# HarmoniaLeo/FRLW-EvD

Hardware: AMD Instinct MI355X
Metric: TAF encode throughput (Mevents/s) (higher is better)
Workload: dtype f32

## Files before the change

### frlw-evd_amd/csrc/taf_column.h

```cpp
#pragma once
#include "frlw_common.h"
#include "taf_plan.h"

namespace {
using namespace frlw;
#define LDS_FENCE() asm volatile("" ::: "memory")
#define LDS_BARRIER() asm volatile("s_waitcnt lgkmcnt(0)\n\ts_barrier" ::: "memory")


struct CmP {
    const uint32_t *dir;
    int n_chunks;
    const uint32_t *rec;
    int TB;
    int chunk_ev;
    uint32_t *hot_start;
    uint32_t *hot_seg0;
    uint32_t *segdesc;
    int max_segs;
};

template <int NT>
__device__ __forceinline__ uint32_t col_load(const CmP &m, const SeqTab &S, int s, int b, uint32_t *L, uint32_t *D, uint32_t *wsum)
{
    constexpr int NWV = NT / kWave;
    const int tid = threadIdx.x, lane = tid & 63, wv = tid >> 6;
    const int c0 = S.chunk0[s], C = S.chunk0[s + 1] - c0;
    const uint32_t out0 = (uint32_t)(S.ev0[s] - S.ev0[0]);
    uint32_t carry = 0;
    for (int cb = 0; cb < C; cb += NT) {
        const int c = cb + tid;
        const uint32_t v = m.dir[(long long)b * m.n_chunks + (c0 + (c < C ? c : C - 1))];
        const uint32_t e = c < C ? v : 0u, cnt = e >> 16;
        const uint32_t inc = wave_incl_scan(cnt);
        if (lane == kWave - 1) wsum[wv] = inc;
        __syncthreads();
        uint32_t run = carry + inc - cnt, total = 0;
#pragma unroll
        for (int k = 0; k < NWV; ++k) { if (k < wv) run += wsum[k]; total += wsum[k]; }
        if (c < C) {
            L[c] = run;
            D[c] = out0 + (uint32_t)c * (uint32_t)m.chunk_ev + (e & 0xffffu) - run;
        }
        carry += total;
        __syncthreads();
    }
    if (tid == 0) L[C] = carry;
    __syncthreads();
    return (uint32_t)__builtin_amdgcn_readfirstlane((int)carry);
}

__device__ __forceinline__ uint32_t col_load_wave(const CmP &m, const SeqTab &S, int s, int b, uint32_t *L, uint32_t *D)
{
    const int lane = threadIdx.x & 63;
    const int c0 = S.chunk0[s], C = S.chunk0[s + 1] - c0;
    const uint32_t out0 = (uint32_t)(S.ev0[s] - S.ev0[0]);
    uint32_t n = 0;
    for (int cb = 0; cb < C; cb += kWave) {
        const int c = cb + lane;
        const uint32_t v = m.dir[(long long)b * m.n_chunks + (c0 + (c < C ? c : C - 1))];
        const uint32_t e = c < C ? v : 0u, cnt = e >> 16;
        const uint32_t inc = wave_incl_scan(cnt), run = n + inc - cnt;
        if (c < C) { L[c] = run; D[c] = out0 + (uint32_t)c * (uint32_t)m.chunk_ev + (e & 0xffffu) - run; }
        n += (uint32_t)__builtin_amdgcn_readlane((int)inc, kWave - 1);
    }
    if (lane == 0) L[C] = n;
    return n;
}

template <int NG, int RU, class Sink>
__device__ __forceinline__ void col_gather(const uint32_t *L, const uint32_t *D, int C, int g16, int l16, const uint32_t *rec, Sink sink)
{
    for (int cc0 = g16; cc0 < C; cc0 += NG * RU) {
        uint32_t v[RU], at[RU], cnt[RU];
#pragma unroll
        for (int u = 0; u < RU; ++u) {
            const int c = cc0 + NG * u, cc = c < C ? c : C - 1;
            const uint32_t lo = L[cc];
            cnt[u] = c < C ? L[cc + 1] - lo : 0u;
            at[u] = lo;
            v[u] = rec[D[cc] + lo + ((uint32_t)l16 < cnt[u] ? (uint32_t)l16 : 0u)];
        }
#pragma unroll
        for (int u = 0; u < RU; ++u) {
            if ((uint32_t)l16 < cnt[u]) sink(at[u] + l16, v[u]);
            if (cnt[u] > 16u) {
                const int c = cc0 + NG * u;
                const uint32_t d = D[c], lo = L[c];
                for (uint32_t j = 16u + l16; j < cnt[u]; j += 16u) sink(lo + j, rec[d + lo + j]);
            }
        }
    }
}

template <int NT>
__device__ __forceinline__ void col_index(const uint32_t *L, int C, uint32_t lo, uint32_t hi, uint16_t *idx)
{
    for (int c = threadIdx.x; c < C; c += NT) {
        const uint32_t a = L[c] > lo ? L[c] : lo, z = L[c + 1] < hi ? L[c + 1] : hi;
        for (uint32_t i = (a + 15u) & ~15u; i < z; i += 16u) idx[(i - lo) >> 4] = (uint16_t)c;
    }
}

__device__ __forceinline__ uint32_t col_addr(const uint32_t *L, const uint32_t *D, uint32_t c, uint32_t i);

__device__ __forceinline__ uint32_t col_addr_wave(const uint32_t *L, const uint32_t *D, const uint16_t *idx, uint32_t lo, uint32_t r0,
                                                  uint32_t ric, uint32_t nr)
{
    if (r0 >= nr) return D[0] + L[0];
    const uint32_t i0 = lo + r0, last = lo + (r0 + 63u < nr ? r0 + 63u : nr - 1u);
    uint32_t cs = (uint32_t)__builtin_amdgcn_readfirstlane((int)idx[r0 >> 4]);
    uint32_t lnext = (uint32_t)__builtin_amdgcn_readfirstlane((int)L[cs + 1]);
    while (lnext <= i0) { ++cs; lnext = (uint32_t)__builtin_amdgcn_readfirstlane((int)L[cs + 1]); }
    if (lnext > last) return (uint32_t)__builtin_amdgcn_readfirstlane((int)D[cs]) + lo + ric;
    return col_addr(L, D, idx[ric >> 4], lo + ric);
}

__device__ __forceinline__ uint32_t col_addr(const uint32_t *L, const uint32_t *D, uint32_t c, uint32_t i)
{
    c += L[c + 1] <= i ? 1u : 0u;
    c += L[c + 1] <= i ? 1u : 0u;
    if (__builtin_expect(__ballot(L[c + 1] <= i) != 0ull, 0))
        while (L[c + 1] <= i) ++c;
    return D[c] + i;
}
}
```

### frlw-evd_amd/csrc/taf_partition.h

```cpp
#pragma once
#include "taf_decode.h"
#include <stddef.h>

namespace {
__host__ __device__ inline uint32_t whole_max_of(int pairs) { return pairs < kFewPairs ? (uint32_t)kSplitSeg : (uint32_t)kSplitWhole; }
__host__ __device__ inline uint32_t split_segments(uint32_t n, uint32_t whole_max) { return n > whole_max ? (n + kSplitSeg - 1) / kSplitSeg : 0u; }

struct HistSpan {
    long long first;
    long long begin, end;
    long long t0;
};

__device__ __forceinline__ HistSpan hist_span(const FastGeom &G, const SeqTab &S, int chunk, int n_chunks)
{
    HistSpan L;
    L.begin = L.end = L.first = 0;
    L.t0 = 0;
    if (chunk >= n_chunks) return L;
    const int s = seq_of_chunk(S, chunk);
    L.t0 = S.t0[s];
    L.begin = S.ev0[s] + (long long)(chunk - S.chunk0[s]) * G.chunk_ev;
    L.end = L.begin + G.chunk_ev < S.ev0[s + 1] ? L.begin + G.chunk_ev : S.ev0[s + 1];
    if (L.end < L.begin) L.end = L.begin;
    L.first = L.begin - (long long)((reinterpret_cast<uintptr_t>(G.data + L.begin) >> 3) & 1u);
    if (L.first < 0) L.first = L.begin;
    return L;
}

__device__ __forceinline__ uint32_t hist_pairs(const HistSpan &L)
{
    long long cover = L.end - L.first;
    if (cover > 2ll * (kMaxBpw / 2) * kFT) cover = 2ll * (kMaxBpw / 2) * kFT;
    return (uint32_t)(cover >> 1);
}

__device__ __forceinline__ void hist_issue(const FastGeom &G, const HistSpan &L, uint4 (&v)[kMaxBpw / 2])
{
    const uint32_t pairs = hist_pairs(L);
    if (pairs > 0) {
        const uint4 *src = (const uint4 *)(G.data + L.first);
#pragma unroll
        for (int j = 0; j < kMaxBpw / 2; ++j) {
            const uint32_t pj = (uint32_t)(j * kFT) + threadIdx.x;
            v[j] = src[pj < pairs ? pj : pairs - 1u];
        }
    }
}

template <bool HAS_MAP, bool EV = false, bool SIMPLE = false>
__global__ __launch_bounds__(kFT) __attribute__((amdgpu_waves_per_eu(8, 8))) void kf_hist(FastGeom G, SeqTab S, uint32_t *counts,
                                                                                         int32_t *errs, float *tlut_w, int n_chunks)
{
    extern __shared__ uint32_t lds[];
    uint32_t *hist = lds;
    __shared__ int serr;
    const int tid = threadIdx.x;
    for (int b = tid; b < G.T; b += kFT) hist[b] = 0;
    if (tid == 0) serr = 0;
    int mul_err = 0;
    if (EV) {
        const double den = (double)G.win, rcp = G.rcp;
        for (long long r = (long long)blockIdx.x * kFT + tid; r <= (long long)G.win; r += (long long)gridDim.x * kFT) {
            const float exact = (float)((double)r / den);
            if ((float)((double)r * rcp) != exact) mul_err = ST_MULBAD;
            tlut_w[r] = exact;
        }
    } else if (tlut_w) {
        const double den = (double)G.win + 1e-8, rcp = G.rcp;
        for (long long r = (long long)blockIdx.x * kFT + tid; r <= (long long)G.win; r += (long long)gridDim.x * kFT) {
            const float exact = (float)((double)r / den);
            if ((float)((double)r * rcp) != exact) mul_err = ST_MULBAD;
            tlut_w[r] = exact - 1.0f;
        }
    }
    uint4 cur[kMaxBpw / 2], nxt[kMaxBpw / 2];
    HistSpan Lc, Ln = hist_span(G, S, (int)blockIdx.x, n_chunks);
    hist_issue(G, Ln, nxt);
    if (mul_err) atomicOr(&serr, mul_err);
    __syncthreads();
    for (int chunk = (int)blockIdx.x; chunk < n_chunks; chunk += (int)gridDim.x) {
        Lc = Ln;
#pragma unroll
        for (int j = 0; j < kMaxBpw / 2; ++j) cur[j] = nxt[j];
        Ln = hist_span(G, S, chunk + (int)gridDim.x, n_chunks);
        hist_issue(G, Ln, nxt);
        int err = 0;
        const uint32_t pairs = hist_pairs(Lc);
        const bool skip_first = Lc.first != Lc.begin;
#pragma unroll
        for (int j = 0; j < kMaxBpw / 2; ++j) {
            const uint32_t pj = (uint32_t)(j * kFT + tid);
            if (pj < pairs && !(skip_first && pj == 0u)) {
                const FastEv o = fast_decode<HAS_MAP, EV, SIMPLE>(G, make_uint2(cur[j].x, cur[j].y), Lc.t0);
                err |= o.err;
                if (o.tile >= 0) atomicAdd(&hist[o.tile], 1u);
            }
            if (pj < pairs) {
                const FastEv o = fast_decode<HAS_MAP, EV, SIMPLE>(G, make_uint2(cur[j].z, cur[j].w), Lc.t0);
                err |= o.err;
                if (o.tile >= 0) atomicAdd(&hist[o.tile], 1u);
            }
        }
        if (tid == 0 && Lc.end > Lc.begin && Lc.first + 2ll * pairs < Lc.end) {
            const FastEv o = fast_decode<HAS_MAP, EV, SIMPLE>(G, G.data[Lc.end - 1], Lc.t0);
            err |= o.err;
            if (o.tile >= 0) atomicAdd(&hist[o.tile], 1u);
        }
        if (err) atomicOr(&serr, err);
        __syncthreads();
        uint32_t *row = counts + (long long)chunk * G.T;
        for (int b = tid; b < G.T; b += kFT) { row[b] = hist[b]; hist[b] = 0u; }
        if (tid == 0) { errs[chunk] = serr; serr = 0; }
        __syncthreads();
    }
}

__device__ __forceinline__ void slabscan_one(const SeqTab &S, uint32_t *counts, int T, uint32_t *slabtot, int slab, int b)
{
    const int s = seq_of(S.slab0, S.n_seq, slab);
    const int c0 = S.chunk0[s] + (slab - S.slab0[s]) * kFastSlab, cend = S.chunk0[s + 1];
    uint32_t v[kFastSlab];
#pragma unroll
    for (int k = 0; k < kFastSlab; ++k) v[k] = (c0 + k < cend) ? counts[(long long)(c0 + k) * T + b] : 0u;
    uint32_t run = 0;
#pragma unroll
    for (int k = 0; k < kFastSlab; ++k) {
        const uint32_t t = v[k];
        v[k] = run;
        run += t;
    }
#pragma unroll
    for (int k = 0; k < kFastSlab; ++k)
        if (c0 + k < cend) counts[(long long)(c0 + k) * T + b] = v[k];
    slabtot[(long long)slab * T + b] = run;
}
__global__ __launch_bounds__(kWave) void kf_slabscan(SeqTab S, uint32_t *counts, int T, uint32_t *slabtot)
{
    const int b = blockIdx.x * kWave + threadIdx.x;
    if (b < T) slabscan_one(S, counts, T, slabtot, blockIdx.y, b);
}

constexpr int kInlineSlabScan = 8192;
__global__ __launch_bounds__(kFT) void kf_tilescan(SeqTab S, uint32_t *slabtot, int T, uint32_t *base, uint32_t *seg0,
                                                   FastHeader *hdr, const int32_t *errs, int chunks, uint32_t *counts_inline,
                                                   int slabs_inline, int no_segments)
{
    if (counts_inline) {
        for (int i = threadIdx.x; i < slabs_inline * T; i += kFT) slabscan_one(S, counts_inline, T, slabtot, i / T, i % T);
        __syncthreads();
    }
    __shared__ uint32_t tot[kMaxPairs];
    __shared__ uint32_t wsum[kFW], wsum2[kFW];
    const int tid = threadIdx.x, lane = tid & 63, wv = tid >> 6;
    const int pairs = S.n_seq * T;
    if (tid == 0) { hdr->status = 0; hdr->filtered_tiles = 0u; hdr->mul_bad = 0u; }
    if (tid < kMaxSeq) hdr->wmask[tid] = 0ull;
    __syncthreads();
    {
        int e = 0;
        for (int c = tid; c < chunks; c += kFT) e |= errs[c];
        if (e & ~ST_MULBAD) atomicOr(&hdr->status, e & ~ST_MULBAD);
        if (e & ST_MULBAD) hdr->mul_bad = 1u;
    }
    const uint32_t whole_max = no_segments ? 0xffffffffu : whole_max_of(pairs);
    uint32_t carry = 0, scarry = 0;
    for (int p0 = 0; p0 < pairs; p0 += kMaxPairs) {
        const int np = pairs - p0 < kMaxPairs ? pairs - p0 : kMaxPairs;
        for (int idx = tid; idx < np; idx += kFT) {
            const int gi = p0 + idx, s = gi / T, b = gi - s * T;
            uint32_t run = 0;
            const int sl1 = S.slab0[s + 1];
            for (int sl = S.slab0[s]; sl < sl1; sl += 8) {
                uint32_t v[8];
#pragma unroll
                for (int k = 0; k < 8; ++k) v[k] = sl + k < sl1 ? slabtot[(long long)(sl + k) * T + b] : 0u;
#pragma unroll
                for (int k = 0; k < 8; ++k) {
                    if (sl + k < sl1) slabtot[(long long)(sl + k) * T + b] = run;
                    run += v[k];
                }
            }
            tot[idx] = run;
        }
        __syncthreads();
        const int per = (np + kFT - 1) / kFT;
        const int b0 = tid * per;
        int b1 = b0 + per;
        if (b1 > np) b1 = np;
        uint32_t sum = 0, ssum = 0;
        for (int b = b0; b < b1; ++b) { sum += tot[b]; ssum += split_segments(tot[b], whole_max); }
        uint32_t inc = sum, sinc = ssum;
#pragma unroll
        for (int off = 1; off < kWave; off <<= 1) {
            const uint32_t v = __shfl_up(inc, off), v2 = __shfl_up(sinc, off);
            if (lane >= off) { inc += v; sinc += v2; }
        }
        if (lane == kWave - 1) { wsum[wv] = inc; wsum2[wv] = sinc; }
        __syncthreads();
        uint32_t pre = 0, spre = 0, all = 0, sall = 0;
        for (int k = 0; k < kFW; ++k) {
            if (k < wv) { pre += wsum[k]; spre += wsum2[k]; }
            all += wsum[k]; sall += wsum2[k];
        }
        uint32_t run = carry + pre + inc - sum, srun = scarry + spre + sinc - ssum;
        for (int b = b0; b < b1; ++b) {
            base[p0 + b] = run;
            seg0[p0 + b] = srun;
            run += tot[b];
            srun += split_segments(tot[b], whole_max);
        }
        carry += all;
        scarry += sall;
        __syncthreads();
    }
    if (tid == 0) { base[pairs] = carry; seg0[pairs] = scarry; }
    if (tid == 0) fold_sticky_status(hdr, hdr->status);
}

template <bool HAS_MAP, bool EV = false, bool SIMPLE = false>
__global__ __launch_bounds__(kFT) void kf_scatter(FastGeom G, SeqTab S, const uint32_t *counts, const uint32_t *slabtot,
                                                  const uint32_t *base, uint32_t *records, FastHeader *hdr)
{
    extern __shared__ uint32_t lds[];
    const int T = G.T;
    uint32_t *wcnt_all = lds;
    uint32_t *loff = wcnt_all + (size_t)kFW * T;
    uint32_t *stage = loff + ((T + 2) & ~1);
    uint16_t *stile = (uint16_t *)(stage + G.chunk_ev);
    __shared__ uint32_t wtot[kFW];
    __shared__ unsigned long long wg_seen;
    const int tid = threadIdx.x, lane = tid & 63, wv = tid >> 6;
    const int chunk = (int)chunk_of_block(blockIdx.x, gridDim.x);
    const int s = seq_of_chunk(S, chunk);
    uint32_t *wcnt = wcnt_all + (size_t)wv * T;
    for (int b = tid; b < kFW * T; b += kFT) wcnt_all[b] = 0;
    if (tid == 0) wg_seen = 0ull;
    __syncthreads();

    const long long chunk_begin = S.ev0[s] + (long long)(chunk - S.chunk0[s]) * G.chunk_ev;
    const long long wave_begin = chunk_begin + (long long)wv * G.run;
    const long long left = S.ev0[s + 1] - wave_begin;
    const uint32_t nloc = left < (long long)G.run ? (uint32_t)(left < 0 ? 0 : left) : (uint32_t)G.run;
    const long long t0 = S.t0[s];
    uint2 q[kMaxBpw];
    if (nloc > 0) {
        const uint2 *src = G.data + wave_begin;
#pragma unroll
        for (int j = 0; j < kMaxBpw; ++j) {
            const uint32_t i = (uint32_t)(j * kWave + lane);
            q[j] = src[i < nloc ? i : nloc - 1u];
        }
    }
    const int slab = S.slab0[s] + (chunk - S.chunk0[s]) / kFastSlab;
    const int tcl = tid < T ? tid : 0;
    const uint32_t gs_a = base[s * T + tcl], gs_b = slabtot[(long long)slab * T + tcl], gs_c = counts[(long long)chunk * T + tcl];
    uint32_t where[kMaxBpw], word[kMaxBpw];
    unsigned long long wseen = 0ull;
#pragma unroll
    for (int j = 0; j < kMaxBpw; ++j) {
        where[j] = 0xffffffffu;
        word[j] = 0u;
        if (j < G.bpw) {
            const uint32_t i = (uint32_t)(j * kWave + lane);
            if (i < nloc) {
                const FastEv o = fast_decode<HAS_MAP, EV, SIMPLE>(G, q[j], t0);
                if (o.tile >= 0) {
                    const uint32_t r = atomicAdd(&wcnt[o.tile], 1u);
                    where[j] = ((uint32_t)o.tile << 16) | r;
                    word[j] = o.word;
                    wseen |= 1ull << o.window;
                }
            }
        }
    }
    __syncthreads();
    uint32_t mine = 0;
    for (int b = tid; b < T; b += kFT) {
        uint32_t run = 0;
#pragma unroll
        for (int w = 0; w < kFW; ++w) {
            const uint32_t v = wcnt_all[(size_t)w * T + b];
            wcnt_all[(size_t)w * T + b] = run;
            run += v;
        }
        mine = run;
    }
    const uint32_t inc = wave_incl_scan(mine);
    if (lane == kWave - 1) wtot[wv] = inc;
    __syncthreads();
    uint32_t pre = 0, total = 0;
#pragma unroll
    for (int k = 0; k < kFW; ++k) { if (k < wv) pre += wtot[k]; total += wtot[k]; }
    if (tid < T) loff[tid] = pre + inc - mine;
    __syncthreads();
#pragma unroll
    for (int j = 0; j < kMaxBpw; ++j) {
        if (j < G.bpw && where[j] != 0xffffffffu) {
            const uint32_t b = where[j] >> 16;
            const uint32_t slot = loff[b] + wcnt[b] + (where[j] & 0xffffu);
            stage[slot] = word[j];
            stile[slot] = (uint16_t)b;
        }
    }
#pragma unroll
    for (int off = 32; off >= 1; off >>= 1) {
        const unsigned lo = __shfl_xor((unsigned)wseen, off), hi = __shfl_xor((unsigned)(wseen >> 32), off);
        wseen |= ((unsigned long long)hi << 32) | lo;
    }
    if (lane == 0 && wseen) atomicOr(&wg_seen, wseen);
    __syncthreads();
    if (tid < T) loff[tid] = (gs_a + gs_b + gs_c) - loff[tid];
    __syncthreads();
    for (uint32_t qi = tid; qi < total; qi += kFT) records[loff[stile[qi]] + qi] = stage[qi];
    if (tid == 0) {
        const unsigned long long m = wg_seen;
        const unsigned long long have = __hip_atomic_load(&hdr->wmask[s], __ATOMIC_RELAXED, __HIP_MEMORY_SCOPE_AGENT);
        if (m & ~have) atomicOr(&hdr->wmask[s], m);
    }
}


#ifndef FRLW_SCATTER_AHEAD
#define FRLW_SCATTER_AHEAD 4
#endif
#if defined(FRLW_WALK_PROF) || defined(FRLW_SCAT_PROF)
constexpr int kProfWgs = 131072;
__device__ unsigned long long g_walk_prof[kProfWgs * 9];
#define XPROF(i) do { const unsigned long long t_ = __builtin_amdgcn_s_memtime(); pd_[i] += t_ - tp_; tp_ = t_; } while (0)
#define XPROF_INIT() unsigned long long tp_ = __builtin_amdgcn_s_memtime(), pd_[9] = {0, 0, 0, 0, 0, 0, 0, 0, 0}
#define XPROF_END() do { if (threadIdx.x == 0 && blockIdx.x < kProfWgs) for (int i_ = 0; i_ < 9; ++i_) g_walk_prof[blockIdx.x * 9 + i_] += pd_[i_]; } while (0)
#endif
#ifdef FRLW_WALK_PROF
#define WPROF(i) XPROF(i)
#define WPROF_INIT() XPROF_INIT()
#define WPROF_END() XPROF_END()
#else
#define WPROF(i) do { } while (0)
#define WPROF_INIT() do { } while (0)
#define WPROF_END() do { } while (0)
#endif
#ifdef FRLW_SCAT_PROF
#define SPROF(i) XPROF(i)
#define SPROF_INIT() XPROF_INIT()
#define SPROF_END() XPROF_END()
#define SPROF_DRAIN() asm volatile("s_waitcnt vmcnt(0)" ::: "memory")
#else
#define SPROF(i) do { } while (0)
#define SPROF_INIT() do { } while (0)
#define SPROF_END() do { } while (0)
#define SPROF_DRAIN() do { } while (0)
#endif
template <bool HAS_MAP, bool EV = false, bool SIMPLE = false, int MAXB = kMaxBpw, int SAE = 0>
__global__ __launch_bounds__(kFT) __attribute__((amdgpu_waves_per_eu(MAXB > kMaxBpw ? 4 : 8, MAXB > kMaxBpw ? 4 : 8))) void kf_scatter_cm(FastGeom G, SeqTab S, uint32_t *dir, uint32_t *records, FastHeader *hdr, float *tlut_w,
                                                     uint32_t epoch)
{
    extern __shared__ uint32_t lds[];
    const int T = G.T;
    uint32_t *wcnt_all = lds;
    uint32_t *loff = wcnt_all + (size_t)kFW * T;
    uint32_t *stage = loff + ((T + 2) & ~1);
    __shared__ uint32_t wtot[kFW];
    __shared__ unsigned long long wg_seen;
    __shared__ int serr;
    constexpr bool LEAN = SIMPLE && !EV && !HAS_MAP && SAE == 0;
    const int tid = threadIdx.x, lane = tid & 63, wv = LEAN ? __builtin_amdgcn_readfirstlane(tid >> 6) : tid >> 6;
    SPROF_INIT();
    const int chunk = (int)chunk_of_block(blockIdx.x, gridDim.x);
    const int s = seq_of_chunk(S, chunk);
    uint32_t *wcnt = wcnt_all + (size_t)wv * T;
    for (int b = tid; b < kFW * T; b += kFT) wcnt_all[b] = 0;
    if (tid == 0) { wg_seen = 0ull; serr = 0; }
    if (blockIdx.x == 0 && epoch != 0u) {
        uint32_t *h32 = (uint32_t *)hdr;
        for (int i = tid; i < (int)(offsetof(FastHeader, epoch) / 4); i += kFT) h32[i] = 0u;
        if (tid == 0) {
            uint32_t *sw = (uint32_t *)((char *)hdr + kStallOffset);
            const uint32_t was = __hip_atomic_load(sw, __ATOMIC_RELAXED, __HIP_MEMORY_SCOPE_AGENT);
            if (was != 0u && was != epoch) atomicCAS(sw, was, 0u);
        }
        __threadfence();
        __syncthreads();
        if (tid == 0) __hip_atomic_store(&hdr->epoch, epoch, __ATOMIC_RELEASE, __HIP_MEMORY_SCOPE_AGENT);
    }

    const long long chunk_begin = S.ev0[s] + (long long)(chunk - S.chunk0[s]) * G.chunk_ev;
    const long long wave_begin = chunk_begin + (long long)wv * G.run;
    const long long left = S.ev0[s + 1] - wave_begin;
    const uint32_t nloc = left < (long long)G.run ? (uint32_t)(left < 0 ? 0 : left) : (uint32_t)G.run;
    const long long t0 = S.t0[s];
    constexpr int kAhead = MAXB > FRLW_SCATTER_AHEAD ? FRLW_SCATTER_AHEAD : MAXB;
    uint2 q[MAXB];
    const uint2 *src = G.data + wave_begin;
    const uint32_t last = nloc - 1u;
    if (nloc > 0) {
#pragma unroll
        for (int j = 0; j < kAhead; ++j) q[j] = src[min((uint32_t)(j * kWave + lane), last)];
    }
    int pre_err = 0;
    if (tlut_w) {
        const double den = EV ? (double)G.win : (double)G.win + 1e-8, rcp = G.rcp;
        bool bad = false;
        for (long long r = (long long)blockIdx.x * kFT + tid; r <= (long long)G.win; r += (long long)gridDim.x * kFT) {
            const float exact = (float)((double)r / den);
            bad |= (float)((double)r * rcp) != exact;
            tlut_w[r] = EV ? exact : exact - 1.0f;
        }
        if (bad) pre_err = ST_MULBAD;
    }
    asm volatile("s_waitcnt lgkmcnt(0)\n\ts_barrier" ::: "memory");
    SPROF(0);
    SPROF(1);
    constexpr bool FASTBLK = LEAN && MAXB > kMaxBpw;
    uint32_t where[MAXB], word[MAXB];
    unsigned long long wseen = 0ull;
    uint32_t wseen32 = 0u;
    int err = pre_err;
    const uint32_t t0lo = (uint32_t)t0;
    const uint32_t nfast = FASTBLK && G.m24 && G.n_windows <= 32 && t0lo <= ~G.span ? nloc >> 6 : 0u;
#pragma unroll
    for (int j = 0; j < MAXB; ++j) {
        where[j] = 0xffffffffu;
        word[j] = 0u;
        if (j + kAhead < MAXB) {
            if (nloc > 0 && j + kAhead < G.bpw)
                q[j + kAhead] = src[min((uint32_t)((j + kAhead) * kWave + lane), last)];
            asm volatile("" ::: "memory");
        }
        bool fast = false;
        uint32_t fx = 0u, fy = 0u, frel = 0u;
        if (FASTBLK && (uint32_t)j < nfast) {
            fx = q[j].y & 16383u; fy = (q[j].y >> 14) & 16383u; frel = q[j].x - t0lo;
            fast = (__builtin_amdgcn_ballot_w64(fx >= (uint32_t)G.W) | __builtin_amdgcn_ballot_w64(fy >= (uint32_t)G.H_full) |
                    __builtin_amdgcn_ballot_w64(frel >= G.span)) == 0ull;
        }
        if (fast) {
            uint32_t tile, w, z;
            simple_taf_fields_valid(G, fx, fy, (q[j].y >> 28) & 1u, frel, tile, w, z);
            const uint32_t r = atomicAdd(&wcnt[tile], 1u);
            wseen32 |= 1u << z;
            word[j] = w;
            where[j] = (tile << 16) | r;
        } else if (j < G.bpw) {
            const uint32_t i = (uint32_t)(j * kWave + lane);
            if (LEAN) {
                if (nloc > 0) {
                    int x = (int)(q[j].y & 16383u), y = (int)((q[j].y >> 14) & 16383u);
                    const uint32_t p = (q[j].y >> 28) & 1u;
                    const bool ib = !fast_alias(G, x, y);
                    uint32_t tile, w, z;
                    const bool sb = !simple_taf_fields<!FASTBLK>(G, x, y, p, q[j].x, t0lo, tile, w, z);
                    const bool live = i < nloc, ok = live && !ib && !sb;
                    if (live && !ok) err |= ib ? ST_INDEX : ST_SPAN;
                    uint32_t r = 0u;
                    if (ok) {
                        r = atomicAdd(&wcnt[tile], 1u);
                        wseen |= 1ull << z;
                    }
                    where[j] = ok ? (tile << 16) | r : 0xffffffffu;
                    word[j] = w;
                }
            } else if (i < nloc) {
                const FastEv o = fast_decode<HAS_MAP, EV, SIMPLE, SAE>(G, q[j], t0);
                err |= o.err;
                if (o.tile >= 0) {
                    const uint32_t r = atomicAdd(&wcnt[o.tile], 1u);
                    where[j] = ((uint32_t)o.tile << 16) | r;
                    word[j] = SAE ? ((uint32_t)(wave_begin - S.ev0[s] + (long long)i + 1) << kCellBits) | (o.word & (uint32_t)(kCells - 1)) : o.word;
                    wseen |= 1ull << o.window;
                }
            }
        }
    }
    wseen |= wseen32;
    if (err) atomicOr(&serr, err);
    SPROF(2);
    __syncthreads();
    SPROF(3);
    uint32_t mine = 0;
    uint32_t pv[kFW];
    {
        const int b = tid < T ? tid : 0;
#pragma unroll
        for (int w = 0; w < kFW; ++w) {
            pv[w] = mine;
            mine += wcnt_all[(size_t)w * T + b];
        }
        if (tid >= T) mine = 0u;
    }
    const uint32_t inc = wave_incl_scan(mine);
    if (lane == kWave - 1) wtot[wv] = inc;
    __syncthreads();
    uint32_t pre = 0, total = 0;
#pragma unroll
    for (int k = 0; k < kFW; ++k) { if (k < wv) pre += wtot[k]; total += wtot[k]; }
    const uint32_t my_off = pre + inc - mine;
    if (tid < T) {
#pragma unroll
        for (int w = 0; w < kFW; ++w) wcnt_all[(size_t)w * T + tid] = pv[w] + my_off;
        dir[(long long)tid * (long long)gridDim.x + chunk] = (mine << 16) | my_off;
    }
    __syncthreads();
    SPROF(4);
#pragma unroll
    for (int j = 0; j < MAXB; ++j) {
        if (j < G.bpw && where[j] != 0xffffffffu) {
            const uint32_t b = where[j] >> 16;
            stage[wcnt[b] + (where[j] & 0xffffu)] = word[j];
        }
    }
#pragma unroll
    for (int off = 32; off >= 1; off >>= 1) {
        const unsigned lo = __shfl_xor((unsigned)wseen, off), hi = __shfl_xor((unsigned)(wseen >> 32), off);
        wseen |= ((unsigned long long)hi << 32) | lo;
    }
    if (lane == 0 && wseen) atomicOr(&wg_seen, wseen);
    __syncthreads();
    SPROF(5);
    uint32_t *dst = records + (chunk_begin - S.ev0[0]);
    uint32_t q4 = 0u;
    if (((reinterpret_cast<uintptr_t>(dst) | reinterpret_cast<uintptr_t>(stage)) & 15u) == 0u) {
        q4 = total & ~3u;
        for (uint32_t qi = 4u * tid; qi < q4; qi += 4u * kFT) *reinterpret_cast<uint4 *>(dst + qi) = *reinterpret_cast<const uint4 *>(stage + qi);
    }
    for (uint32_t qi = q4 + tid; qi < total; qi += kFT) dst[qi] = stage[qi];
    SPROF(6);
    SPROF_DRAIN();
    SPROF(7);
    SPROF_END();
    if (tid == 0) {
        if (epoch != 0u) {
            uint32_t polls = 0u;
            while (__hip_atomic_load(&hdr->epoch, __ATOMIC_ACQUIRE, __HIP_MEMORY_SCOPE_AGENT) != epoch) {
                if (++polls > (1u << 22)) break;
                __builtin_amdgcn_s_sleep(2);
            }
            if (polls > (1u << 22)) {
                atomicExch((uint32_t *)((char *)hdr + kStallOffset), epoch);
                fold_sticky_status(hdr, ST_STALL);
                return;
            }
        }
        const unsigned long long m = wg_seen;
        const unsigned long long have = __hip_atomic_load(&hdr->wmask[s], __ATOMIC_RELAXED, __HIP_MEMORY_SCOPE_AGENT);
        if (m & ~have) atomicOr(&hdr->wmask[s], m);
        const int e = serr;
        if (e & ~ST_MULBAD) { atomicOr(&hdr->status, e & ~ST_MULBAD); fold_sticky_status(hdr, e & ~ST_MULBAD); }
        if (e & ST_MULBAD) hdr->mul_bad = 1u;
    }
}
}
```

### frlw-evd_amd/csrc/taf_split.h

```cpp
#pragma once
#include "taf_blocktab.h"
#include "taf_column.h"
#include "taf_partition.h"
#include <type_traits>

namespace {
struct TileP {
    int H, W, twl, thl, tiles_x, T, K, n_windows, wb, flip;
    uint32_t win;
    const uint32_t *rec;
    uint32_t *rec2;
    const uint32_t *base;
    uint32_t *sub;
    uint32_t *sub_end;
    const uint32_t *seg0;
    uint32_t *segcnt;
    int pairs;
    int direct;
    int seg_grid;
    uint32_t tile_max;
    const float *tlut;
    const uint32_t *leaky_thr;
    FastHeader *hdr;
    double rcp;
    float *state;
    float *view_f32;
    uint8_t *out_u8;
    uint32_t *wst, *wst_flag;
};

__device__ __forceinline__ int pair_of_segment(const uint32_t *seg0, int pairs, uint32_t seg)
{
    int lo = 0, hi = pairs;
    while (hi - lo > 1) {
        const int mid = (lo + hi) >> 1;
        if (seg0[mid] <= seg) lo = mid; else hi = mid;
    }
    return lo;
}

__device__ __forceinline__ void count_subtiles(const uint32_t *rec, uint32_t beg, uint32_t end, uint32_t (*wtot)[kFW])
{
    const int tid = threadIdx.x, wv = tid >> 6;
    for (uint32_t c0 = beg; c0 < end; c0 += 8 * kFT) {
        uint32_t v[8];
#pragma unroll
        for (int u = 0; u < 8; ++u) {
            const uint32_t i = c0 + (uint32_t)(u * kFT + tid);
            v[u] = rec[i < end ? i : end - 1u];
        }
#pragma unroll
        for (int u = 0; u < 8; ++u)
            if (c0 + (uint32_t)(u * kFT + tid) < end) atomicAdd(&wtot[wv][(v[u] & (kCells - 1)) >> 8], 1u);
    }
}

__device__ __forceinline__ void split_count_segment(const TileP &q, uint32_t seg, uint32_t (*wtot)[kFW])
{
    const int tid = threadIdx.x, wv = tid >> 6;
    if (seg >= q.seg0[q.pairs]) return;
    const int g = pair_of_segment(q.seg0, q.pairs, seg);
    const uint32_t beg = q.base[g] + (seg - q.seg0[g]) * (uint32_t)kSplitSeg;
    const uint32_t end = q.base[g + 1] - beg < (uint32_t)kSplitSeg ? q.base[g + 1] : beg + kSplitSeg;
    if (tid < kFW * kFW) (&wtot[0][0])[tid] = 0u;
    __syncthreads();
    count_subtiles(q.rec, beg, end, wtot);
    __syncthreads();
    if (tid < kFW) {
        uint32_t t = 0;
#pragma unroll
        for (int w = 0; w < kFW; ++w) t += wtot[w][tid];
        q.segcnt[(long long)seg * kFW + tid] = t;
    }
}

constexpr int kWholeChunks = FRLW_WHOLE_SEGS;
constexpr int kWholeBatches = kWholeChunks * kSplitSeg / kWave;
constexpr int kWholeRow = kWholeBatches + 1;

template <bool CM>
__global__ __launch_bounds__(kFT) __attribute__((amdgpu_waves_per_eu(8, 8))) void kf_split_whole(TileP q, CmP cm, SeqTab S)
{
    constexpr int RPT = kSplitSeg / kFT;
    constexpr int kBtGroup = 4;
    constexpr int kColWords = 2 * kColMax + 1 + kSplitWhole / 32 + 1;
    constexpr int kPoolTail = CM && kColWords > kSplitSeg ? kColWords - kSplitSeg : 0;
    __shared__ __attribute__((aligned(16))) uint32_t pool[kFW * kWholeRow + kSplitSeg + kPoolTail];
    uint32_t *scnt = pool, *stage = pool + kFW * kWholeRow;
    __shared__ uint32_t wtot[kFW][kFW];
    __shared__ uint32_t vtot[kFW];
    __shared__ uint32_t vbeg[kFW][kFW];
    __shared__ uint32_t cE[kFW][kFW], cD[kFW][kFW];
    __shared__ uint32_t s_start, s_first;
    __shared__ int s_unsorted;
    __shared__ int s_fw[kWholeChunks][kFW], s_lw[kWholeChunks][kFW];
    __shared__ uint32_t s_wst[CM ? kFW * (FRLW_MAX_WINDOWS + 1) : 1];
    const int tid = threadIdx.x, lane = tid & 63, wv = tid >> 6;
    const int32_t status0 = q.hdr->status;
    if (!CM && status0 != 0) return;
    const int blk = (int)blockIdx.x;
    if (!CM && blk >= q.pairs) {
        const uint32_t nseg = q.seg0[q.pairs];
        for (uint32_t seg = (uint32_t)(blk - q.pairs); seg < nseg; seg += (uint32_t)q.seg_grid) {
            split_count_segment(q, seg, wtot);
            __syncthreads();
        }
        return;
    }
    const int g = CM ? (int)xcd_owned_index(blockIdx.x, gridDim.x) : blk;
    uint32_t beg, n;
    uint32_t m[kWholeChunks][RPT];
    if (CM) {
        const int s = g / q.T, C = S.chunk0[s + 1] - S.chunk0[s];
        const bool tabled = C <= frlw_bt::kBtCols && S.ev0[S.n_seq] - S.ev0[0] < (1ll << 28);
        static_assert(2 * frlw_bt::kBtCols + 2 + kSplitWhole / 16 * 2 <= kSplitSeg, "column + table inside the staging area");
        uint32_t *colL = stage, *colD = stage + (tabled ? frlw_bt::kBtCols : kColMax) + 1;
        uint16_t *idx = (uint16_t *)(stage + 2 * kColMax + 1);
        frlw_bt::BtEntry *tab = (frlw_bt::BtEntry *)(stage + 2 * frlw_bt::kBtCols + 2);
        for (int i = tid; i < kFW * kWholeRow; i += kFT) scnt[i] = 0u;
        n = col_load<kFT>(cm, S, s, g - s * q.T, colL, colD, &wtot[0][0]);
        if (status0 != 0) return;
        if (n == 0u) {
            if (tid < kFW) { q.sub[(long long)g * kFW + tid] = 0u; q.sub_end[(long long)g * kFW + tid] = 0u; }
            if (q.wst && tid == 0) q.wst_flag[g] = 0u;
            return;
        }
        const bool hot = n > q.tile_max;
        if (tid == 0) {
            s_start = atomicAdd(&q.hdr->rec_cursor, n);
            if (hot) s_first = atomicAdd(&q.hdr->seg_cursor, (n + kSplitSeg - 1) / kSplitSeg);
            if (q.wst && hot) q.wst_flag[g] = 0u;
            s_unsorted = 0;
        }
        if (q.wst && !hot) {
            if (tid < kWholeChunks * kFW) { (&s_fw[0][0])[tid] = -1; (&s_lw[0][0])[tid] = -1; }
            for (int i = tid; i < kFW * (q.n_windows + 1); i += kFT) s_wst[i] = 0xffffffffu;
        }
        if (hot) {
            __syncthreads();
            const uint32_t nseg = (n + kSplitSeg - 1) / kSplitSeg, first = s_first;
            if (tid == 0) { cm.hot_start[g] = s_start; cm.hot_seg0[g] = first; }
            for (uint32_t k = tid; k < nseg; k += kFT)
                if (first + k < (uint32_t)cm.max_segs) cm.segdesc[first + k] = (uint32_t)g;
            return;
        }
        if (tabled) {
            for (int c = tid; c < C; c += kFT) frlw_bt::bt_build_run(colL, colD, C, c, n, tab);
        } else {
            col_index<kFT>(colL, C, 0u, n, idx);
        }
        __syncthreads();
        const uint32_t wvs = (uint32_t)__builtin_amdgcn_readfirstlane(wv);
        {
            const __amdgpu_buffer_rsrc_t rsrc = __builtin_amdgcn_make_buffer_rsrc((void *)cm.rec, 0, 0xffffffffu, 0x00020000);
            if (tabled) {
#pragma unroll
                for (int c = 0; c < kWholeChunks; ++c) {
                    if ((uint32_t)(c * kSplitSeg) >= n) break;
#pragma unroll
                    for (int u0 = 0; u0 < RPT; u0 += kBtGroup) {
                        frlw_bt::BtEntry e[kBtGroup];
                        uint32_t ic[kBtGroup], wmax = 0u;
#pragma unroll
                        for (int k = 0; k < kBtGroup; ++k) {
                            const uint32_t i = (uint32_t)(c * kSplitSeg + (u0 + k) * kFT + tid);
                            ic[k] = i < n ? i : n - 1u;
                            e[k] = tab[ic[k] >> 4];
                        }
#pragma unroll
                        for (int k = 0; k < kBtGroup; ++k) wmax = e[k].w > wmax ? e[k].w : wmax;
                        if (__builtin_expect(__ballot(wmax == frlw_bt::kBtFallback) == 0ull, 1)) {
#pragma unroll
                            for (int k = 0; k < kBtGroup; ++k)
                                m[c][u0 + k] = (uint32_t)__builtin_amdgcn_raw_buffer_load_b32(rsrc, (int)(frlw_bt::bt_addr(e[k], ic[k]) << 2), 0, 0);
                        } else {
#pragma unroll
                            for (int k = 0; k < kBtGroup; ++k) {
                                const uint32_t off = e[k].w == frlw_bt::kBtFallback ? frlw_bt::bt_walk(colL, colD, e[k].a, ic[k]) : frlw_bt::bt_addr(e[k], ic[k]);
                                m[c][u0 + k] = (uint32_t)__builtin_amdgcn_raw_buffer_load_b32(rsrc, (int)(off << 2), 0, 0);
                            }
                        }
                    }
                }
            } else {
#pragma unroll
            for (int c = 0; c < kWholeChunks; ++c) {
                if ((uint32_t)(c * kSplitSeg) >= n) break;
#pragma unroll
                for (int u = 0; u < RPT; ++u) {
                    const uint32_t i = (uint32_t)(c * kSplitSeg + u * kFT + tid), ic = i < n ? i : n - 1u;
                    const uint32_t i0 = (uint32_t)(c * kSplitSeg + u * kFT) + wvs * kWave;
                    uint32_t off = 0u;
                    if (i0 < n) {
                        const uint32_t last = i0 + 63u < n ? i0 + 63u : n - 1u;
                        uint32_t cs = (uint32_t)__builtin_amdgcn_readfirstlane((int)idx[i0 >> 4]);
                        uint32_t lnext = (uint32_t)__builtin_amdgcn_readfirstlane((int)colL[cs + 1]);
                        while (lnext <= i0) { ++cs; lnext = (uint32_t)__builtin_amdgcn_readfirstlane((int)colL[cs + 1]); }
                        if (lnext > last) off = (uint32_t)__builtin_amdgcn_readfirstlane((int)colD[cs]) + ic;
                        else off = col_addr(colL, colD, idx[ic >> 4], ic);
                    }
                    m[c][u] = (uint32_t)__builtin_amdgcn_raw_buffer_load_b32(rsrc, (int)(off << 2), 0, 0);
                }
            }
            }
        }
        beg = (uint32_t)__builtin_amdgcn_readfirstlane((int)s_start);
    } else {
        beg = q.base[g];
        const uint32_t end = q.base[g + 1];
        if (g == q.pairs - 1 && tid == 0) q.sub[(long long)q.pairs * kFW] = end;
        if (end - beg > whole_max_of(q.pairs)) return;
        n = end - beg;
        if (n == 0u) {
            if (tid < kFW) q.sub[(long long)g * kFW + tid] = beg;
            return;
        }
#pragma unroll
        for (int c = 0; c < kWholeChunks; ++c)
#pragma unroll
            for (int u = 0; u < RPT; ++u) {
                const uint32_t i = (uint32_t)(c * kSplitSeg + u * kFT + tid);
                m[c][u] = q.rec[beg + (i < n ? i : n - 1u)];
            }
    }
    if (!CM) {
        for (int i = tid; i < kFW * kWholeRow; i += kFT) scnt[i] = 0u;
        __syncthreads();
    }
    uint32_t rk[kWholeChunks][RPT / 4];
#pragma unroll
    for (int c = 0; c < kWholeChunks; ++c) {
#pragma unroll
        for (int u4 = 0; u4 < RPT / 4; ++u4) rk[c][u4] = 0u;
#pragma unroll
        for (int u = 0; u < RPT; ++u) {
            const uint32_t i0 = (uint32_t)(c * kSplitSeg + u * kFT + wv * kWave);
            if (i0 < n) {
                const bool valid = i0 + (uint32_t)lane < n;
                const uint32_t b = valid ? (m[c][u] & (kCells - 1)) >> 8 : (uint32_t)(lane & 15);
                const uint32_t t = atomicAdd(&scnt[b * kWholeRow + (c * RPT + u) * kFW + wv], valid ? 1u : 0u);
                rk[c][u >> 2] |= t << (8 * (u & 3));
            }
        }
    }
    __syncthreads();
    {
        uint32_t carry = 0;
#pragma unroll
        for (int k = 0; k < kWholeBatches / kWave; ++k) {
            if ((uint32_t)(k * kWave * kWave) < n) {
                const uint32_t v = scnt[wv * kWholeRow + k * kWave + lane];
                const uint32_t inc = wave_incl_scan(v);
                scnt[wv * kWholeRow + k * kWave + lane] = carry + inc - v;
                carry += __shfl(inc, kWave - 1);
            }
        }
        if (lane == 0) vtot[wv] = carry;
    }
    __syncthreads();
    {
        const uint32_t t = vtot[lane & 15];
        uint32_t inc = t;
#pragma unroll
        for (int o2 = 1; o2 < kFW; o2 <<= 1) {
            const uint32_t u = __shfl_up(inc, o2);
            if ((lane & 15) >= o2) inc += u;
        }
        if (lane < kFW) {
            vbeg[wv][lane] = beg + inc - t;
            if (wv == 0) {
                q.sub[(long long)g * kFW + lane] = beg + inc - t;
                if (CM) q.sub_end[(long long)g * kFW + lane] = beg + inc;
            }
        }
        LDS_FENCE();
    }
    const bool wtab = CM && q.wst != nullptr;
#pragma unroll
    for (int c = 0; c < kWholeChunks; ++c) {
        if ((uint32_t)(c * kSplitSeg) >= n) break;
        const uint32_t nch = n - (uint32_t)(c * kSplitSeg) < (uint32_t)kSplitSeg ? n - (uint32_t)(c * kSplitSeg) : (uint32_t)kSplitSeg;
        {
            const int b = lane & 15;
            const uint32_t p0 = scnt[b * kWholeRow + c * (kSplitSeg / kWave)];
            const uint32_t p1 = (uint32_t)((c + 1) * kSplitSeg) < n ? scnt[b * kWholeRow + (c + 1) * (kSplitSeg / kWave)] : vtot[b];
            const uint32_t cnt = p1 - p0;
            uint32_t inc = cnt;
#pragma unroll
            for (int o2 = 1; o2 < kFW; o2 <<= 1) {
                const uint32_t u = __shfl_up(inc, o2);
                if (b >= o2) inc += u;
            }
            if (lane < kFW) {
                cE[wv][lane] = (inc - cnt) - p0;
                cD[wv][lane] = vbeg[wv][lane] + p0 - (inc - cnt);
            }
            LDS_FENCE();
        }
#pragma unroll
        for (int u = 0; u < RPT; ++u) {
            const uint32_t i = (uint32_t)(u * kFT + tid);
            if (i < nch) {
                const uint32_t b = (m[c][u] & (kCells - 1)) >> 8;
                const uint32_t t = (rk[c][u >> 2] >> (8 * (u & 3))) & 255u;
                stage[cE[wv][b] + scnt[b * kWholeRow + (c * RPT + u) * kFW + wv] + t] = m[c][u];
            }
        }
        __syncthreads();
#pragma unroll
        for (int u = 0; u < RPT; ++u) {
            const uint32_t i = (uint32_t)(u * kFT + tid);
            if (i < nch) {
                const uint32_t r = stage[i];
                q.rec2[cD[wv][(r & (kCells - 1)) >> 8] + i] = r;
            }
        }
        if (wtab) {
            const uint32_t dmask = (((1u << q.wb) - 1u) << kCellBits) | (uint32_t)(kCells - 1) >> 8 << 8;
            uint32_t cand = 0u;
#pragma unroll
            for (int u0 = 0; u0 < RPT; u0 += 2) {
                uint32_t r[2], rp[2];
#pragma unroll
                for (int k = 0; k < 2; ++k) {
                    const uint32_t i = (uint32_t)((u0 + k) * kFT + tid);
                    r[k] = stage[i];
                    rp[k] = stage[(i - 1u) & (kSplitSeg - 1)];
                }
#pragma unroll
                for (int k = 0; k < 2; ++k) asm volatile("" : "+v"(r[k]), "+v"(rp[k]));
#pragma unroll
                for (int k = 0; k < 2; ++k) {
                    const uint32_t i = (uint32_t)((u0 + k) * kFT + tid);
                    cand |= (i < nch && (((r[k] ^ rp[k]) & dmask) != 0u || i == 0u || i == nch - 1u) ? 1u : 0u) << (u0 + k);
                }
            }
            while (cand) {
                const int u = __builtin_ctz(cand);
                cand &= cand - 1u;
                const uint32_t i = (uint32_t)(u * kFT + tid);
                const uint32_t r = stage[i], rp = stage[i > 0u ? i - 1u : 0u];
                const int bsub = (int)((r & (kCells - 1)) >> 8), bp = (int)((rp & (kCells - 1)) >> 8);
                const int wc = (int)__builtin_amdgcn_ubfe(r, kCellBits, q.wb), wpn = (int)__builtin_amdgcn_ubfe(rp, kCellBits, q.wb);
                const bool same = i > 0u && bp == bsub;
                if (!same || wc != wpn) atomicMin(&s_wst[bsub * (q.n_windows + 1) + wc], cD[wv][bsub] + i - vbeg[wv][bsub]);
                if (same && wc < wpn) s_unsorted = 1;
                if (!same) { s_fw[c][bsub] = wc; if (i > 0u) s_lw[c][bp] = wpn; }
                if (i == nch - 1u) s_lw[c][bsub] = wc;
            }
        }
        if (wtab && (uint32_t)((c + 1) * kSplitSeg) >= n) LDS_BARRIER();
        else __syncthreads();
    }
    if (wtab) {
        if (tid < kFW) {
            int prev = -1;
            for (int c = 0; c < kWholeChunks; ++c)
                if (s_fw[c][tid] >= 0) { if (s_fw[c][tid] < prev) s_unsorted = 1; prev = s_lw[c][tid]; }
        }
        uint32_t *const wr = q.wst + (long long)g * kFW * (q.n_windows + 1);
        for (int i = tid; i < kFW * (q.n_windows + 1); i += kFT) wr[i] = s_wst[i];
        LDS_BARRIER();
        if (tid == 0) q.wst_flag[g] = s_unsorted ? 2u : 1u;
    }
}

constexpr int kSplitRpt = kSplitSeg / kFT;
struct PlaceLds {
    uint32_t scnt[kSplitRpt][kFW][kFW];
    uint32_t vtot[kFW];
    uint32_t stot[kFW], sdst[kFW];
    uint32_t cE[kFW][kFW], cD[kFW][kFW];
    uint32_t stage[kSplitSeg];
};

struct ColLds {
    uint32_t L[kColMax + 1], D[kColMax];
    uint16_t idx[kSplitSeg / 16];
    uint32_t wsum[kFW + 1];
};

template <bool CM>
__device__ __forceinline__ void split_place_segment(const TileP &q, uint32_t seg, PlaceLds &L, const CmP &cm, const SeqTab &S, ColLds *cl)
{
    constexpr int RPT = kSplitRpt, NE = RPT * kFW;
    const int tid = threadIdx.x, lane = tid & 63, wv = tid >> 6;
    int g;
    uint32_t beg, nrec, seg_first, seg_last, tile_start;
    if (CM) {
        g = __builtin_amdgcn_readfirstlane((int)cm.segdesc[seg]);
        const int s = g / q.T;
        const uint32_t n = col_load<kFT>(cm, S, s, g - s * q.T, cl->L, cl->D, cl->wsum);
        seg_first = (uint32_t)__builtin_amdgcn_readfirstlane((int)cm.hot_seg0[g]);
        seg_last = seg_first + (n + kSplitSeg - 1) / kSplitSeg;
        beg = (seg - seg_first) * (uint32_t)kSplitSeg;
        nrec = n - beg < (uint32_t)kSplitSeg ? n - beg : (uint32_t)kSplitSeg;
        tile_start = (uint32_t)__builtin_amdgcn_readfirstlane((int)cm.hot_start[g]);
        col_index<kFT>(cl->L, S.chunk0[s + 1] - S.chunk0[s], beg, beg + nrec, cl->idx);
    } else {
        g = pair_of_segment(q.seg0, q.pairs, seg);
        beg = q.base[g] + (seg - q.seg0[g]) * (uint32_t)kSplitSeg;
        const uint32_t end = q.base[g + 1] - beg < (uint32_t)kSplitSeg ? q.base[g + 1] : beg + kSplitSeg;
        nrec = end - beg;
        seg_first = q.seg0[g];
        seg_last = q.seg0[g + 1];
        tile_start = q.base[g];
    }
    for (int i = tid; i < RPT * kFW * kFW; i += kFT) (&L.scnt[0][0][0])[i] = 0u;
    uint32_t before = 0, total = 0;
    for (uint32_t sg = seg_first + lane; sg < seg_last; sg += kWave) {
        const uint32_t c = q.segcnt[(long long)sg * kFW + wv];
        total += c;
        if (sg < seg) before += c;
    }
#pragma unroll
    for (int o2 = 32; o2 >= 1; o2 >>= 1) { before += __shfl_xor(before, o2); total += __shfl_xor(total, o2); }
    if (lane == 0) L.vtot[wv] = total;
    __syncthreads();
    uint32_t vstart = tile_start;
    for (int k = 0; k < wv; ++k) vstart += L.vtot[k];
    if (seg == seg_first && lane == 0) {
        q.sub[(long long)g * kFW + wv] = vstart;
        if (CM) q.sub_end[(long long)g * kFW + wv] = vstart + total;
    }
    uint32_t m[RPT], rk[RPT];
    const uint32_t wvs = (uint32_t)__builtin_amdgcn_readfirstlane(wv);
#pragma unroll
    for (int u = 0; u < RPT; ++u) {
        const uint32_t i = (uint32_t)(u * kFT + tid);
        if (CM) {
            const uint32_t ic = i < nrec ? i : nrec - 1u;
            const uint32_t v = cm.rec[col_addr_wave(cl->L, cl->D, cl->idx, beg, (uint32_t)(u * kFT) + wvs * kWave, ic, nrec)];
            m[u] = i < nrec ? v : 0u;
        } else {
            m[u] = i < nrec ? q.rec[beg + i] : 0u;
        }
    }
#pragma unroll
    for (int u = 0; u < RPT; ++u) {
        const uint32_t i = (uint32_t)(u * kFT + tid);
        rk[u] = 0u;
        if (i < nrec) rk[u] = atomicAdd(&L.scnt[u][wv][(m[u] & (kCells - 1)) >> 8], 1u);
    }
    __syncthreads();
    {
        uint32_t v0 = 0, v1 = 0;
        const int e0 = 2 * lane, e1 = 2 * lane + 1;
        if (e0 < NE) v0 = L.scnt[e0 / kFW][e0 % kFW][wv];
        if (e1 < NE) v1 = L.scnt[e1 / kFW][e1 % kFW][wv];
        const uint32_t inc = wave_incl_scan(v0 + v1);
        const uint32_t ex = inc - (v0 + v1);
        if (e0 < NE) L.scnt[e0 / kFW][e0 % kFW][wv] = ex;
        if (e1 < NE) L.scnt[e1 / kFW][e1 % kFW][wv] = ex + v0;
        if (lane == kWave - 1) { L.stot[wv] = inc; L.sdst[wv] = vstart + before; }
    }
    __syncthreads();
    {
        const int b = lane & 15;
        const uint32_t cnt = L.stot[b];
        uint32_t inc = cnt;
#pragma unroll
        for (int o2 = 1; o2 < kFW; o2 <<= 1) {
            const uint32_t u = __shfl_up(inc, o2);
            if (b >= o2) inc += u;
        }
        if (lane < kFW) { L.cE[wv][lane] = inc - cnt; L.cD[wv][lane] = L.sdst[lane] - (inc - cnt); }
        LDS_FENCE();
    }
#pragma unroll
    for (int u = 0; u < RPT; ++u) {
        const uint32_t i = (uint32_t)(u * kFT + tid);
        if (i < nrec) {
            const uint32_t b = (m[u] & (kCells - 1)) >> 8;
            L.stage[L.cE[wv][b] + L.scnt[u][wv][b] + rk[u]] = m[u];
        }
    }
    __syncthreads();
#pragma unroll
    for (int u = 0; u < RPT; ++u) {
        const uint32_t i = (uint32_t)(u * kFT + tid);
        if (i < nrec) {
            const uint32_t r = L.stage[i];
            q.rec2[L.cD[wv][(r & (kCells - 1)) >> 8] + i] = r;
        }
    }
}

template <bool CM>
__global__ __launch_bounds__(kFT) __attribute__((amdgpu_waves_per_eu(8, 8))) void kf_split_place(TileP q, CmP cm, SeqTab S)
{
    __shared__ PlaceLds L;
    __shared__ typename std::conditional<CM, ColLds, uint32_t>::type clmem;
    ColLds *cl = reinterpret_cast<ColLds *>(&clmem);
    if (q.hdr->status != 0) return;
    uint32_t nseg = CM ? q.hdr->seg_cursor : q.seg0[q.pairs];
    if (CM && nseg > (uint32_t)cm.max_segs) nseg = (uint32_t)cm.max_segs;
    for (uint32_t seg = blockIdx.x; seg < nseg; seg += gridDim.x) {
        split_place_segment<CM>(q, seg, L, cm, S, cl);
        __syncthreads();
    }
}

__global__ __launch_bounds__(kFT) __attribute__((amdgpu_waves_per_eu(8, 8))) void kf_segcount_cm(TileP q, CmP cm, SeqTab S)
{
    __shared__ ColLds cl;
    __shared__ uint32_t wtot[kFW][kFW];
    const int tid = threadIdx.x, wv = tid >> 6;
    if (q.hdr->status != 0) return;
    uint32_t nseg = q.hdr->seg_cursor;
    if (nseg > (uint32_t)cm.max_segs) nseg = (uint32_t)cm.max_segs;
    for (uint32_t seg = blockIdx.x; seg < nseg; seg += gridDim.x) {
        const int g = __builtin_amdgcn_readfirstlane((int)cm.segdesc[seg]), s = g / q.T;
        const uint32_t n = col_load<kFT>(cm, S, s, g - s * q.T, cl.L, cl.D, cl.wsum);
        const uint32_t beg = (seg - (uint32_t)__builtin_amdgcn_readfirstlane((int)cm.hot_seg0[g])) * (uint32_t)kSplitSeg;
        const uint32_t nrec = n - beg < (uint32_t)kSplitSeg ? n - beg : (uint32_t)kSplitSeg;
        col_index<kFT>(cl.L, S.chunk0[s + 1] - S.chunk0[s], beg, beg + nrec, cl.idx);
        if (tid < kFW * kFW) (&wtot[0][0])[tid] = 0u;
        __syncthreads();
        uint32_t v[kSplitRpt];
        const uint32_t wvs = (uint32_t)__builtin_amdgcn_readfirstlane(wv);
#pragma unroll
        for (int u = 0; u < kSplitRpt; ++u) {
            const uint32_t i = (uint32_t)(u * kFT + tid), ic = i < nrec ? i : nrec - 1u;
            v[u] = cm.rec[col_addr_wave(cl.L, cl.D, cl.idx, beg, (uint32_t)(u * kFT) + wvs * kWave, ic, nrec)];
        }
#pragma unroll
        for (int u = 0; u < kSplitRpt; ++u)
            if ((uint32_t)(u * kFT + tid) < nrec) atomicAdd(&wtot[wv][(v[u] & (kCells - 1)) >> 8], 1u);
        __syncthreads();
        if (tid < kFW) {
            uint32_t t = 0;
#pragma unroll
            for (int w = 0; w < kFW; ++w) t += wtot[w][tid];
            q.segcnt[(long long)seg * kFW + tid] = t;
        }
        __syncthreads();
    }
}
}
```

Baseline: 80730.

## Defer cursor atomic result, use DPP row scans, add split-phase profiling

```diff
diff --git a/frlw-evd_amd/csrc/taf_column.h b/frlw-evd_amd/csrc/taf_column.h
--- a/frlw-evd_amd/csrc/taf_column.h
+++ b/frlw-evd_amd/csrc/taf_column.h
@@ -24,7 +24,7 @@
 __device__ __forceinline__ uint32_t col_load(const CmP &m, const SeqTab &S, int s, int b, uint32_t *L, uint32_t *D, uint32_t *wsum)
 {
     constexpr int NWV = NT / kWave;
-    const int tid = threadIdx.x, lane = tid & 63, wv = tid >> 6;
+    const int tid = threadIdx.x, lane = tid & 63, wv = tid >> 6, wvs = __builtin_amdgcn_readfirstlane(wv);
     const int c0 = S.chunk0[s], C = S.chunk0[s + 1] - c0;
     const uint32_t out0 = (uint32_t)(S.ev0[s] - S.ev0[0]);
     uint32_t carry = 0;
@@ -35,9 +35,9 @@
         const uint32_t inc = wave_incl_scan(cnt);
         if (lane == kWave - 1) wsum[wv] = inc;
         __syncthreads();
-        uint32_t run = carry + inc - cnt, total = 0;
-#pragma unroll
-        for (int k = 0; k < NWV; ++k) { if (k < wv) run += wsum[k]; total += wsum[k]; }
+        const uint32_t ws = lane < NWV ? wsum[lane] : 0u, wsi = wave_incl_scan(ws);
+        const uint32_t total = (uint32_t)__builtin_amdgcn_readlane((int)wsi, NWV - 1);
+        const uint32_t run = carry + inc - cnt + (uint32_t)__builtin_amdgcn_readlane((int)(wsi - ws), wvs);
         if (c < C) {
             L[c] = run;
             D[c] = out0 + (uint32_t)c * (uint32_t)m.chunk_ev + (e & 0xffffu) - run;
diff --git a/frlw-evd_amd/csrc/taf_partition.h b/frlw-evd_amd/csrc/taf_partition.h
--- a/frlw-evd_amd/csrc/taf_partition.h
+++ b/frlw-evd_amd/csrc/taf_partition.h
@@ -323,6 +323,10 @@
 
 #ifndef FRLW_SCATTER_AHEAD
 #define FRLW_SCATTER_AHEAD 4
+#endif
+#if defined(FRLW_SPLIT_PROF) && !defined(FRLW_WALK_PROF) && !defined(FRLW_SCAT_PROF)
+#define FRLW_SCAT_PROF
+#define FRLW_SCAT_PROF_READER_ONLY
 #endif
 #if defined(FRLW_WALK_PROF) || defined(FRLW_SCAT_PROF)
 constexpr int kProfWgs = 131072;
@@ -340,7 +344,7 @@
 #define WPROF_INIT() do { } while (0)
 #define WPROF_END() do { } while (0)
 #endif
-#ifdef FRLW_SCAT_PROF
+#if defined(FRLW_SCAT_PROF) && !defined(FRLW_SCAT_PROF_READER_ONLY)
 #define SPROF(i) XPROF(i)
 #define SPROF_INIT() XPROF_INIT()
 #define SPROF_END() XPROF_END()
@@ -350,6 +354,19 @@
 #define SPROF_INIT() do { } while (0)
 #define SPROF_END() do { } while (0)
 #define SPROF_DRAIN() do { } while (0)
+#endif
+#ifdef FRLW_SPLIT_PROF
+#define PPROF(i) XPROF(i)
+#define PPROF_INIT() XPROF_INIT()
+#define PPROF_END() XPROF_END()
+#define PPROF_CURSOR(n) do {  \
+        if ((n) <= 8192u) __builtin_amdgcn_s_waitcnt(0x0F78); else if ((n) <= 16384u) __builtin_amdgcn_s_waitcnt(0x4F70); \
+        else if ((n) <= 24576u) __builtin_amdgcn_s_waitcnt(0x4F78); else __builtin_amdgcn_s_waitcnt(0x8F70); } while (0)
+#else
+#define PPROF(i) do { } while (0)
+#define PPROF_INIT() do { } while (0)
+#define PPROF_END() do { } while (0)
+#define PPROF_CURSOR(n) do { } while (0)
 #endif
 template <bool HAS_MAP, bool EV = false, bool SIMPLE = false, int MAXB = kMaxBpw, int SAE = 0>
 __global__ __launch_bounds__(kFT) __attribute__((amdgpu_waves_per_eu(MAXB > kMaxBpw ? 4 : 8, MAXB > kMaxBpw ? 4 : 8))) void kf_scatter_cm(FastGeom G, SeqTab S, uint32_t *dir, uint32_t *records, FastHeader *hdr, float *tlut_w,
diff --git a/frlw-evd_amd/csrc/taf_split.h b/frlw-evd_amd/csrc/taf_split.h
--- a/frlw-evd_amd/csrc/taf_split.h
+++ b/frlw-evd_amd/csrc/taf_split.h
@@ -74,6 +74,16 @@
     }
 }
 
+__device__ __forceinline__ uint32_t row16_incl_scan(uint32_t v)
+{
+    static_assert(kFW == 16, "one DPP row per set of sub-tile counters");
+    v += (uint32_t)__builtin_amdgcn_update_dpp(0, (int)v, 0x111, 0xf, 0xf, false);
+    v += (uint32_t)__builtin_amdgcn_update_dpp(0, (int)v, 0x112, 0xf, 0xf, false);
+    v += (uint32_t)__builtin_amdgcn_update_dpp(0, (int)v, 0x114, 0xf, 0xf, false);
+    v += (uint32_t)__builtin_amdgcn_update_dpp(0, (int)v, 0x118, 0xf, 0xf, false);
+    return v;
+}
+
 constexpr int kWholeChunks = FRLW_WHOLE_SEGS;
 constexpr int kWholeBatches = kWholeChunks * kSplitSeg / kWave;
 constexpr int kWholeRow = kWholeBatches + 1;
@@ -108,7 +118,8 @@
         return;
     }
     const int g = CM ? (int)xcd_owned_index(blockIdx.x, gridDim.x) : blk;
-    uint32_t beg, n;
+    PPROF_INIT();
+    uint32_t beg = 0u, n;
     uint32_t m[kWholeChunks][RPT];
     if (CM) {
         const int s = g / q.T, C = S.chunk0[s + 1] - S.chunk0[s];
@@ -119,6 +130,7 @@
         frlw_bt::BtEntry *tab = (frlw_bt::BtEntry *)(stage + 2 * frlw_bt::kBtCols + 2);
         for (int i = tid; i < kFW * kWholeRow; i += kFT) scnt[i] = 0u;
         n = col_load<kFT>(cm, S, s, g - s * q.T, colL, colD, &wtot[0][0]);
+        PPROF(0);
         if (status0 != 0) return;
         if (n == 0u) {
             if (tid < kFW) { q.sub[(long long)g * kFW + tid] = 0u; q.sub_end[(long long)g * kFW + tid] = 0u; }
@@ -126,10 +138,16 @@
             return;
         }
         const bool hot = n > q.tile_max;
+        uint32_t start = 0u;
         if (tid == 0) {
-            s_start = atomicAdd(&q.hdr->rec_cursor, n);
-            if (hot) s_first = atomicAdd(&q.hdr->seg_cursor, (n + kSplitSeg - 1) / kSplitSeg);
-            if (q.wst && hot) q.wst_flag[g] = 0u;
+            uint32_t zero = 0u;
+            asm volatile("" : "+v"(zero));
+            start = atomicAdd(&q.hdr->rec_cursor + zero, n);
+            if (hot) {
+                s_start = start;
+                s_first = atomicAdd(&q.hdr->seg_cursor, (n + kSplitSeg - 1) / kSplitSeg);
+                if (q.wst) q.wst_flag[g] = 0u;
+            }
             s_unsorted = 0;
         }
         if (q.wst && !hot) {
@@ -150,6 +168,7 @@
             col_index<kFT>(colL, C, 0u, n, idx);
         }
         __syncthreads();
+        PPROF(2);
         const uint32_t wvs = (uint32_t)__builtin_amdgcn_readfirstlane(wv);
         {
             const __amdgpu_buffer_rsrc_t rsrc = __builtin_amdgcn_make_buffer_rsrc((void *)cm.rec, 0, 0xffffffffu, 0x00020000);
@@ -202,9 +221,13 @@
                     m[c][u] = (uint32_t)__builtin_amdgcn_raw_buffer_load_b32(rsrc, (int)(off << 2), 0, 0);
                 }
             }
-            }
-        }
-        beg = (uint32_t)__builtin_amdgcn_readfirstlane((int)s_start);
+            __builtin_amdgcn_s_waitcnt(0x0F70);
+            }
+        }
+        PPROF(3);
+        PPROF_CURSOR(n);
+        PPROF(1);
+        if (tid == 0) { asm volatile("" : "+v"(start)); s_start = start; }
     } else {
         beg = q.base[g];
         const uint32_t end = q.base[g + 1];
@@ -243,6 +266,7 @@
             }
         }
     }
+    if (CM) PPROF(4);
     __syncthreads();
     {
         uint32_t carry = 0;
@@ -258,14 +282,11 @@
         if (lane == 0) vtot[wv] = carry;
     }
     __syncthreads();
+    if (CM) PPROF(5);
+    if (CM) beg = (uint32_t)__builtin_amdgcn_readfirstlane((int)s_start);
     {
         const uint32_t t = vtot[lane & 15];
-        uint32_t inc = t;
-#pragma unroll
-        for (int o2 = 1; o2 < kFW; o2 <<= 1) {
-            const uint32_t u = __shfl_up(inc, o2);
-            if ((lane & 15) >= o2) inc += u;
-        }
+        const uint32_t inc = row16_incl_scan(t);
         if (lane < kFW) {
             vbeg[wv][lane] = beg + inc - t;
             if (wv == 0) {
@@ -285,12 +306,7 @@
             const uint32_t p0 = scnt[b * kWholeRow + c * (kSplitSeg / kWave)];
             const uint32_t p1 = (uint32_t)((c + 1) * kSplitSeg) < n ? scnt[b * kWholeRow + (c + 1) * (kSplitSeg / kWave)] : vtot[b];
             const uint32_t cnt = p1 - p0;
-            uint32_t inc = cnt;
-#pragma unroll
-            for (int o2 = 1; o2 < kFW; o2 <<= 1) {
-                const uint32_t u = __shfl_up(inc, o2);
-                if (b >= o2) inc += u;
-            }
+            const uint32_t inc = row16_incl_scan(cnt);
             if (lane < kFW) {
                 cE[wv][lane] = (inc - cnt) - p0;
                 cD[wv][lane] = vbeg[wv][lane] + p0 - (inc - cnt);
@@ -307,6 +323,7 @@
             }
         }
         __syncthreads();
+        if (CM) PPROF(6);
 #pragma unroll
         for (int u = 0; u < RPT; ++u) {
             const uint32_t i = (uint32_t)(u * kFT + tid);
@@ -351,6 +368,7 @@
         }
         if (wtab && (uint32_t)((c + 1) * kSplitSeg) >= n) LDS_BARRIER();
         else __syncthreads();
+        if (CM) PPROF(7);
     }
     if (wtab) {
         if (tid < kFW) {
@@ -363,6 +381,7 @@
         LDS_BARRIER();
         if (tid == 0) q.wst_flag[g] = s_unsorted ? 2u : 1u;
     }
+    if (CM) { PPROF(8); PPROF_END(); }
 }
 
 constexpr int kSplitRpt = kSplitSeg / kFT;
```

Result: faster. 82000 (median of 6 runs) (+1.6%).
